# duckietown/gym-duckietown

Hardware: AMD Instinct MI355X
Metric: env-steps/sec (4096 envs, 640x480 RGB) at 1/2/4/8 MI355X; % HBM roofline (higher is better)
Workload: dtype f32 raster -> u8 frames; f64 physics

## Files before the change

gym-duckietown_amd/csrc/dtsim_dev.h:

```cpp
#pragma once
#include <hip/hip_runtime.h>
#include <stdint.h>
#include "../../include/dtsim.h"
#include "ipm_project.h"
#include "observe_plan.h"
#include "scene_tables.h"
#include "state_fields.h"

#define DT_CAMERA_FORWARD_DIST 0.066
#define DT_ROBOT_WIDTH (0.13 + 0.02)
#define DT_ROBOT_LENGTH 0.18
#define DT_CENTER_SHIFT (DT_CAMERA_FORWARD_DIST - (DT_ROBOT_LENGTH / 2))
#define DT_SAFETY_RAD_MULT 1.8
#define DT_AGENT_SAFETY_RAD ((DT_ROBOT_LENGTH / 2) * DT_SAFETY_RAD_MULT)
#define DT_REWARD_INVALID_POSE (-1000.0)

struct StepParams {
  int32_t n_steps, frame_skip, max_steps, delay_steps;
  int32_t action_mode, actions_f64, auto_reset, n_pool;
  uint32_t step_flags;
  int32_t light_capture, domain_rand;
  int32_t lanes;
  int32_t camera_rand;
  const dtsim_reset_sampler* sampler;
// ... 6 lines not shown
void dt_launch_reset(hipStream_t s, const SimArrays& A, const MapSet& M, const StepParams& P,
                     const uint8_t* mask, const dtsim_init_state* states);
void dt_launch_query(hipStream_t s, const SimArrays& A, const MapSet& M, const StepParams& P, int n,
                     const int32_t* env_idx, const double* poses, double safety_factor, dtsim_probe* out);

struct alignas(16) ScreenTri {
  float bx0, bx1, by0, by1;
  float sx[3], sy[3], iw[3];
  float inv_area;
  int32_t index;
  int32_t pad;
  float cw[3][3];
  float uw[3], vw[3];
  int32_t tex;
};
static_assert(sizeof(ScreenTri) == 128, "ScreenTri is 128 bytes");
struct ObjBox { float bx0, bx1, by0, by1; int32_t first, count, pad[2]; };

#ifndef DT_WAVE_W
#define DT_WAVE_W 128
#endif
#ifndef DT_PPT
#define DT_PPT 4
#endif
#ifndef DT_V3_WW
#define DT_V3_WW 128
#endif
#define DT_TILE_W DT_WAVE_W
#define DT_TILE_H (4 * (64 * DT_PPT / DT_WAVE_W))
#ifndef DT_ENVS_PER_BLOCK
#define DT_ENVS_PER_BLOCK 64
#endif
#ifndef DT_ITEM_B
#define DT_ITEM_B 8
#endif
#define DT_ITEMS_PER_WG (4 * (DT_PPT * DT_ENVS_PER_BLOCK) / DT_ITEM_B)
static inline size_t dt_raster_tiles(int W, int H) {
  return (size_t)((W + DT_TILE_W - 1) / DT_TILE_W) * (size_t)((H + DT_TILE_H - 1) / DT_TILE_H);
}
static inline size_t dt_raster_groups(int N, int W, int H) { return dt_raster_tiles(W, H) * (((size_t)N + DT_ENVS_PER_BLOCK - 1) / DT_ENVS_PER_BLOCK); }

struct RenderParams {
  int32_t N, W, H, distortion;
  int32_t domain_rand, n_maps, n_tile_recs;
  int32_t tex_w, tex_h;
  const TileLds* tile_recs;
  uint8_t* frames;
  const float* lut;
  const uint32_t* texels;
  const TexDev* tex;
  const RenderMapDev* maps;
  const uint32_t* tiles;
  const ObjInstDev* objs;
  const MeshDev* meshes;
  const TriDev* tris;
  void* envcam;
  int32_t max_tris, segment;
  ScreenTri* stris;
  float4* tribox;
  ObjBox* objbox;
  float* blockbox;
  unsigned long long* objmask;
  uint2* objrange;
  uint16_t* queue;
  int32_t* qcount;
  uint16_t* qend;
  int32_t* work;
  uint32_t* items;
  uint32_t* items2;
  const uint8_t* mesh_seg;
  const uint8_t* qtex;
  const uint32_t* qtiles;
  int32_t n_qtiles, qlog2;
  float q_per_m;
  int32_t qmax_tiles;
  int32_t* envpos;
  void* dump;
  void* pixtab;
  void* envv;
  void* envd;
  int32_t q3_rows;
  int32_t light;
};
#define DT_WORK_INTS 8
#define DT_WORK_ITEMS 0
#define DT_WORK_CURSOR 1
#define DT_WORK_OBJ_FRONT 2
#define DT_WORK_OBJ_CURSOR 3
#define DT_WORK_OBJ_BACK 6
#define DT_WORK_LIVE 7
struct RenderDump { uint8_t store[64 * 16]; };
enum RenderSlab { DT_SLAB_ENV, DT_SLAB_PIX, DT_SLAB_QUEUE, DT_SLAB_QCOUNT, DT_SLAB_ITEMS, DT_SLAB_QEND, DT_SLAB_STRIS, DT_SLAB_OBJBOX, DT_SLAB_OBJMASK, DT_SLABS };
void dt_render_layout(int N, int W, int H, int max_tris, size_t* bytes, void* const* base = nullptr, RenderParams* R = nullptr);
int dt_raster_pipe(RenderParams& R, int grid_rows, int grid_cols, bool raster_old);
int dt_launch_render(hipStream_t s, const SimArrays& A, const RenderParams& R, int pipe, int tables, const uint8_t* mask = nullptr);
void dt_launch_overlay_lines(hipStream_t s, const RenderParams& R, const float* d_lines, int first, int count, int env);
void dt_launch_overlay_leds(hipStream_t s, const RenderParams& R, const float* d_spheres, int first, int count, int env);
void dt_launch_depth(hipStream_t s, const RenderParams& R, void* out, int oh, int ow, bool f16, const uint8_t* mask);
void dt_launch_labels(hipStream_t s, const RenderParams& R, const uint8_t* texel_class, const uint8_t* mesh_class, int n_mesh_class, uint8_t* out,
                      uint8_t* inst, int oh, int ow, const uint8_t* mask);
void dt_launch_bev(hipStream_t s, const RenderParams& R, const SimArrays& A, const double* ocorners, const uint8_t* texel_class,
                   const uint8_t* mesh_class, int n_mesh_class, uint8_t* cls, uint8_t* inst, int oh, int ow, double cell, int rows_behind,
                   const uint8_t* mask);
struct IpmArgs {
  const uint8_t* frames;
  int N, W, H;
  uint8_t *img, *valid;
  int32_t* src;
  int oh, ow;
  double cell;
  int rows_behind;
  bool chw;
  const uint8_t* mask;
};
void dt_launch_ipm_table(hipStream_t s, int32_t* table, const IpmCal* cal, int W, int H, int oh, int ow, double cell, int rows_behind);
void dt_launch_ipm_gather(hipStream_t s, const IpmArgs& a, const int32_t* table);
void dt_launch_ipm_env(hipStream_t s, const IpmArgs& a, const SimArrays& A, bool per_env, const IpmCal* cals, int n_cal, const int32_t* env_cal);
void dt_launch_remap_cal(hipStream_t s, const uint8_t* scratch, uint8_t* frames, const int32_t* src, const int32_t* env_cal,
                         const uint8_t* mask, int N, int W, int H);
void dt_build_remap_maps(int W, int H, int n_cal, const double* K, const double* D, const double* ir, float* rx, float* ry);
void dt_fill_pack_remap(int W, int H, int n_cal, float* rx, float* ry, const int32_t* order, const int64_t* order_off, int32_t* src_index);

void dt_launch_observe(hipStream_t s, const ObservePlan& plan, const ObserveParams& P, const uint8_t* mask = nullptr);
void dt_launch_copy_rows(hipStream_t s, int N, void* dst, const void* src, size_t row_bytes, const uint8_t* mask);
void dt_launch_boxes(hipStream_t s, int N, const uint8_t* inst, int oh, int ow, int32_t* out, const uint8_t* mask);
void dt_launch_obs_push(hipStream_t s, int N, void* stack, const uint8_t* obs, int depth, int out_h, int out_w, bool f32, bool gray,
                        const uint8_t* first, const uint8_t* mask);
struct BlendArgs {
  const uint8_t* f[DTSIM_BLEND_MAX];
  uint32_t w[DTSIM_BLEND_MAX];
  int n;
};
void dt_launch_blend_frames(hipStream_t s, int N, void* out, const BlendArgs& B, size_t frame_bytes, bool f32, const uint8_t* mask);
```

gym-duckietown_amd/csrc/render.hip:

```cpp
#include "dtsim_dev.h"
#include <hip/hip_fp16.h>
#include <type_traits>
#include <algorithm>
#include <map>
#include <mutex>
#include <tuple>

typedef int v3_i32x4 __attribute__((ext_vector_type(4)));
typedef uint32_t v3_u32x3 __attribute__((ext_vector_type(3)));
__device__ void v3_buf_store_v3i32(v3_u32x3 data, v3_i32x4 rsrc, int voffset, int soffset, int aux) __asm("llvm.amdgcn.raw.buffer.store.v3i32");
typedef uint32_t v3_u32x4 __attribute__((ext_vector_type(4)));
__device__ void v3_buf_store_v4i32(v3_u32x4 data, v3_i32x4 rsrc, int voffset, int soffset, int aux) __asm("llvm.amdgcn.raw.buffer.store.v4i32");
#define V3_RSRC_W3 0x00027000
__device__ inline v3_i32x4 v3_rsrc(const void* p, uint32_t bytes) {
  v3_i32x4 r;
  r.x = (int)(uint32_t)reinterpret_cast<uintptr_t>(p); r.y = (int)((reinterpret_cast<uintptr_t>(p) >> 32) & 0xFFFFu); r.z = (int)bytes; r.w = V3_RSRC_W3;
  return r;
}


#define RB 256
#define PPT DT_PPT
#define WAVE_W DT_WAVE_W
#define SLOT_X(k, l) (((k) * 64 + (l)) % WAVE_W)
#define SLOT_Y(k, l) (((k) * 64 + (l)) / WAVE_W)
#define WAVE_PIX (64 * PPT)
#define ENVS_PER_BLOCK DT_ENVS_PER_BLOCK
#ifndef DT_TRI_CAP
#define DT_TRI_CAP 96
#endif
#ifndef DT_TRI_PAD
#define DT_TRI_PAD 0.5f
#endif
#define TRI_CAP DT_TRI_CAP

#define CLS_SKY 0
#define CLS_GROUND 1
#define CLS_TILE 2

#define NEAR_Z 0.04f
#define FAR_Z 100.0f
#define GROUND_Y (-0.008f)
#define GROUND_HALF 50.0f

struct alignas(16) EnvCam {
  float Cx, Cy, Cz;
  float sa, ca;
  float sth, cth;
  float tx, ty;
  float hor[3];
  float gnd[3];
  float base[3];
  float dif[3];
  float L[4];
  float gndl[4];
  int32_t map_id;
  float pad[2];
};
static_assert(sizeof(EnvCam) == 128, "EnvCam is 128 bytes");

struct alignas(16) EnvFast {
  float A, B, Cxi, Czi;
  float kg, Cx, Cz, its;
  float ts, gw_m, gh_m, I0;
  uint32_t hor_rgb;
  int32_t gw, gh, tile_off;
};
static_assert(sizeof(EnvFast) == 64, "EnvFast is 64 bytes");

struct alignas(16) EnvQ {
  float A, B, Cx, Cz;
  float Xhi, Zhi;
  uint32_t tab_b, pitch4;
  uint32_t hor_rgb;
  uint32_t sky[3];
  uint32_t reach;
  uint32_t env;
  uint32_t pad[2];
};
static_assert(sizeof(EnvQ) == 64, "EnvQ is 64 bytes");
struct alignas(16) EnvV {
  float A2[2], B2[2], Cx2[2], Cz2[2];
  float Xhi, Zhi;
// ... 853 lines not shown
}

__device__ inline PixInv pix_inv_dr(float nx, float ny, bool valid, const DrCam& d, const float L[4]) {
  PixInv p;
  p.flags = valid ? PF_VALID : 0u;
  p.lr = p.lf = p.ndl = p.mrg = 0.f;
  const float xe = nx * d.tx, yla = fmaf(ny, d.a1, -d.sth), fwd = fmaf(ny, d.a2, d.cth);
  if (!(yla < 0.f)) {
    p.flags |= (yla - d.dy >= 0.f) ? PF_SKY : PF_ALWAYS_EDGE;
    return p;
  }
  const float inv = frcp(-yla);
  const float t = d.Cy * inv;
  p.lr = t * xe; p.lf = t * fwd;
  if (d.directional) p.ndl = d.ndl_dir;
  else { Ray r; r.xe = xe; r.ye = ny * d.ty; r.yla = yla; r.fwd = fwd; p.ndl = plane_ndl(L, d.sth, d.cth, r, t); }
  const float rho = d.dy * inv;
  const float kappa = fmaf(rho * 1.3334f, rho, rho);
  const float sx = fmaf(fabsf(p.lr), kappa, t * d.cex), fy = fmaf(fabsf(p.lf), kappa, t * d.eys);
  p.mrg = 1.05f * fsqrt_(fmaf(sx, sx, fy * fy));
  const float tg = t * d.kgc;
  if (t >= NEAR_Z && t <= FAR_Z) p.flags |= PF_TILE_OK;
  if (tg >= NEAR_Z && tg <= FAR_Z) p.flags |= PF_GROUND_OK;
  if (rho > 0.25f || tg * (1.f + 2.f * rho) > FAR_Z * 0.98f || t * (1.f - 2.f * rho) < NEAR_Z * 1.02f)
    p.flags |= PF_ALWAYS_EDGE;
  return p;
}

#define QREGION (WAVE_PIX * ENVS_PER_BLOCK)
#define QE_PLANE_EDGE 0x8000u
__device__ inline int qe_pixel(const uint32_t ent) { return (int)(ent & 255u); }
__device__ inline int qe_envpos(const uint32_t ent) { return (int)((ent >> 8) & 63u); }
__device__ inline bool qe_plane_edge(const uint32_t ent) { return (ent & QE_PLANE_EDGE) != 0u; }
static_assert(ENVS_PER_BLOCK <= 64, "the env position of a queue entry has six bits");
#define ITEM_B DT_ITEM_B
#define ITEMS_PER_WG DT_ITEMS_PER_WG
#define GRAB_MAX 16
#ifndef DT_RES_ENVS
#define DT_RES_ENVS 1
#endif
#define RES_ENVS DT_RES_ENVS
static_assert(ENVS_PER_BLOCK % RES_ENVS == 0 && ENVS_PER_BLOCK / RES_ENVS <= ITEMS_PER_WG, "octet items");

__device__ inline int dt_sub_live(const RenderParams& R) { return __builtin_amdgcn_readfirstlane(R.work[DT_WORK_LIVE]); }
__device__ inline size_t obj_items_cap(const RenderParams& R) {
  const int n_tiles = ((R.W + DT_TILE_W - 1) / DT_TILE_W) * ((R.H + DT_TILE_H - 1) / DT_TILE_H);
  return (size_t)((R.N + ENVS_PER_BLOCK - 1) / ENVS_PER_BLOCK) * n_tiles * (ENVS_PER_BLOCK / RES_ENVS);
}
typedef unsigned long long envmask_t;
__device__ inline void push_obj_items(const RenderParams& R, uint32_t rwg, envmask_t groups = ~0ull, envmask_t heavy = 0ull) {
  const int ng = ENVS_PER_BLOCK / RES_ENVS;
  if (ng < 64) groups &= (1ull << ng) - 1ull;
  heavy &= groups;
  const envmask_t light = groups & ~heavy;
  const int nh = __popcll(heavy), nl = __popcll(light);
  if (nh) {
    int pos = atomicAdd(R.work + DT_WORK_OBJ_FRONT, nh);
    for (int i = 0; i < ng; ++i) if ((heavy >> i) & 1ull) R.items2[pos++] = rwg * ITEMS_PER_WG + (uint32_t)i;
  }
  if (nl) {
    size_t pos = obj_items_cap(R) - 1 - (size_t)atomicAdd(R.work + DT_WORK_OBJ_BACK, nl);
    for (int i = 0; i < ng; ++i) if ((light >> i) & 1ull) R.items2[pos--] = rwg * ITEMS_PER_WG + (uint32_t)i;
  }
}
#ifndef DT_RO_HEAVY
#define DT_RO_HEAVY 128
#endif
__device__ inline envmask_t obj_groups_of(int qend_v, int lane, envmask_t* heavy = nullptr) {
  static_assert(ENVS_PER_BLOCK / RES_ENVS <= 64, "one bit per env group");
  const int up = __shfl_up(qend_v, 1);
  const int cnt = lane < ENVS_PER_BLOCK ? qend_v - (lane == 0 ? 0 : up) : 0;
  const unsigned long long m = __ballot(cnt != 0), mh = __ballot(cnt >= DT_RO_HEAVY);
  envmask_t g = 0ull, gh = 0ull;
#pragma unroll
  for (int i = 0; i < ENVS_PER_BLOCK / RES_ENVS; ++i) {
    g |= ((m >> (i * RES_ENVS)) & ((1ull << RES_ENVS) - 1ull)) ? (1ull << i) : 0ull;
    gh |= ((mh >> (i * RES_ENVS)) & ((1ull << RES_ENVS) - 1ull)) ? (1ull << i) : 0ull;
  }
  if (heavy) *heavy = gh;
  return g;
}


#ifndef DT_Q_TILE_SPLIT
#define DT_Q_TILE_SPLIT 2
#endif
__host__ __device__ inline int dt_q_tile_group(int n_tiles) { return (n_tiles + DT_Q_TILE_SPLIT - 1) / DT_Q_TILE_SPLIT; }
inline size_t raster_wg_grid(size_t n_tiles, int n_chunks) {
  const int q_tg = dt_q_tile_group((int)n_tiles);
  return ((n_tiles + q_tg - 1) / q_tg) * q_tg * ((n_chunks + 7) / 8) * 8;
}
struct RasterWg {
  int NL, tile, chunk; bool live;
  __device__ int rwg(const int n_tiles) const { return chunk * n_tiles + tile; }
  __device__ int e0() const { return chunk * ENVS_PER_BLOCK; }
  __device__ int e1() const { return min(e0() + ENVS_PER_BLOCK, NL); }
};
template <bool SUB, bool SCALAR>
__device__ inline RasterWg raster_wg(const RenderParams& R, const int n_tiles, const unsigned bx) {
  RasterWg w;
  w.NL = SUB ? dt_sub_live(R) : R.N;
  const int n_chunks = (w.NL + ENVS_PER_BLOCK - 1) / ENVS_PER_BLOCK, cpx = (n_chunks + 7) / 8;
  const int xcd = bx & 7, bi = bx >> 3;
  const int q_tg = dt_q_tile_group(n_tiles);
  const int per_group = q_tg * cpx;
  const int grp = bi / per_group, gi = bi % per_group;
  const int g_tiles = min(q_tg, n_tiles - grp * q_tg);
  const int tile = SUB ? (int)bx % n_tiles : grp * q_tg + gi % g_tiles;
  w.tile = SCALAR ? __builtin_amdgcn_readfirstlane(tile) : tile;
  const int chunk = SUB ? (int)bx / n_tiles : xcd * cpx + gi / g_tiles;
  w.chunk = SCALAR ? __builtin_amdgcn_readfirstlane(chunk) : chunk;
  w.live = SUB ? w.chunk < n_chunks : (gi < g_tiles * cpx && w.chunk < n_chunks);
  return w;
}

#define V3_TAB_PITCH 256
#define V3_MAP_COLS 32
__device__ inline void v3_fill_tile_table(const RenderParams& R, const uint32_t* __restrict__ qtiles, uint32_t* s_qt, const int tid) {
  for (int i = tid; i < R.q3_rows * V3_TAB_PITCH; i += RB) s_qt[i] = 0u;
  __syncthreads();
  for (int mi = 0; mi < R.n_maps; ++mi) {
    const int pitch = R.maps[mi].qt_pitch, off = R.maps[mi].qt_off, n = pitch * (R.maps[mi].grid_h + 2 * DT_QRING);
    for (int i = tid; i < n; i += RB) {
      const int r = i / pitch, c = i - r * pitch;
      const uint2 te = reinterpret_cast<const uint2*>(qtiles)[off + i];
      s_qt[r * V3_TAB_PITCH + mi * V3_MAP_COLS + c] = te.x;
      s_qt[r * V3_TAB_PITCH + V3_TAB_PITCH / 2 + mi * V3_MAP_COLS + c] = te.y;
    }
  }
}

__device__ inline void fill_tile_recs(const RenderParams& R, uint32_t* s_mem, const int tid) {
  const uint32_t* src = reinterpret_cast<const uint32_t*>(R.tile_recs);
  for (int i = tid; i < R.n_tile_recs * (int)(sizeof(TileLds) / 4); i += RB) s_mem[i] = src[i];
}

__device__ inline float med3f(float x, float lo, float hi) { return __builtin_amdgcn_fmed3f(x, lo, hi); }
__device__ inline bool v3_sample_owner(const float Xs, const float Zs, const float lo, const float Xhi, const float Zhi, const char* qtb,
                                       const uint32_t tab, uint32_t& tb, uint32_t& sel) {
  const float Xo = Xs - 0.5f, Zo = Zs - 0.5f;
  const float Xc = med3f(Xo, lo, Xhi), Zc = med3f(Zo, lo, Zhi);
  const uint32_t ta = (__builtin_amdgcn_perm((uint32_t)flr_i32(Zc), (uint32_t)flr_i32(Xc), 0x0c0c0501u) << 2) + tab;
  const uint32_t* tp = reinterpret_cast<const uint32_t*>(qtb + ta);
  tb = tp[0]; sel = tp[V3_TAB_PITCH / 2];
  return (Xc == Xo) & (Zc == Zo);
}
__device__ inline float ground_quad_at(const float kg, const float X, const float C) { return fmaf(kg, X - C, C); }
__device__ inline bool ground_quad_in(const float G, const float goff, const float ghalf) { return fabsf(G - goff) <= ghalf; }

__device__ inline int work_n_grabs(const int n_items) {
  const int grab = max(1, min(GRAB_MAX, n_items / (int)(gridDim.x * (RB / 64) * 4)));
  return (n_items + grab - 1) / grab;
}
__device__ inline int work_next_grab(const RenderParams& R, const int cursor, int g, const int lane) {
  if (lane == 0) g = (int)gridDim.x * (RB / 64) + atomicAdd(R.work + cursor, 1);
  return __builtin_amdgcn_readfirstlane(g);
}

template <bool OBJ>
struct ChunkObjMasks {
  static_assert(ENVS_PER_BLOCK <= 64, "one lane per env of the chunk");
  uint32_t lo, hi;
  int e0;
  __device__ void load(const RenderParams& R, const int e0_, const int e1, const int n_blk, const int blk, const int lane) {
    uint32_t om_lo = 0u, om_hi = 0u;
    if (OBJ && lane < e1 - e0_) {
      const unsigned long long v = R.objmask[(size_t)(e0_ + lane) * n_blk + blk];
      om_lo = (uint32_t)v; om_hi = (uint32_t)(v >> 32);
    }
    lo = om_lo; hi = om_hi; e0 = e0_;
  }
  __device__ unsigned long long of(const int e) const {
    if (!OBJ) return 0ull;
    return ((unsigned long long)(uint32_t)__builtin_amdgcn_readlane((int)hi, e - e0) << 32) | (uint32_t)__builtin_amdgcn_readlane((int)lo, e - e0);
  }
};

__device__ inline uint32_t spxy_pack(const float4& l, const int W, const int H) {
  const float sx = (l.x + 1.f) * 0.5f * (float)W, sy = (1.f - l.y) * 0.5f * (float)H;
  return (uint32_t)__half_as_ushort(__float2half(sx)) | ((uint32_t)__half_as_ushort(__float2half(sy)) << 16);
}
__device__ inline void spxy_unpack(uint32_t t, float& sx, float& sy) {
  asm volatile("" : "+v"(t));
  sx = __half2float(__ushort_as_half((unsigned short)(t & 0xFFFFu)));
  sy = __half2float(__ushort_as_half((unsigned short)(t >> 16)));
}

struct alignas(4) U3 { uint32_t a, b, c; };

template <bool DR, bool OBJ>
__global__ __launch_bounds__(RB) void k_raster(RenderParams R, const EnvCam* __restrict__ cams,
                                               const EnvFast* __restrict__ fasts, uint8_t* __restrict__ frames, const uint32_t* __restrict__ texels,
                                               const float4* __restrict__ lut, const RenderMapDev* __restrict__ maps,
                                               const TileLds* __restrict__ tile_recs, uint16_t* __restrict__ queue,
                                               int32_t* __restrict__ qcount) {
  extern __shared__ uint32_t s_mem[];
// ... 1632 lines not shown
}

void dt_launch_ipm_env(hipStream_t s, const IpmArgs& a, const SimArrays& A, bool per_env, const IpmCal* cals, int n_cal, const int32_t* env_cal) {
  if (a.N <= 0) return;
  const bool vec = dt_ipm_vec(a);
  auto k = a.chw ? (vec ? k_ipm_env<true, true> : k_ipm_env<true, false>) : (vec ? k_ipm_env<false, true> : k_ipm_env<false, false>);
  hipLaunchKernelGGL(k, dt_ipm_grid(a), dim3(256), 0, s, a.frames, A.angle, A.cam, per_env ? 1 : 0, dt_ipm_shared_camera(a.W, a.H), cals, n_cal, env_cal,
                     a.N, a.W, a.H, a.oh, a.ow, a.cell, a.rows_behind, a.img, a.valid, a.src, a.mask);
}

void dt_launch_overlay_lines(hipStream_t s, const RenderParams& R, const float* d_lines, int first, int count, int env) {
  if (count <= 0) return;
  hipLaunchKernelGGL(k_overlay_lines, dim3((unsigned)((R.W * R.H + 255) / 256)), dim3(256), 0, s, R, reinterpret_cast<const EnvCam*>(R.envcam), d_lines, first, count, env);
}

template <class K> static size_t resident_blocks(K kernel, size_t lds) {
  static std::mutex mu;
  static std::map<std::tuple<int, size_t, const void*>, size_t> cache;
  int dev = 0;
  (void)hipGetDevice(&dev);
  std::lock_guard<std::mutex> lk(mu);
  const auto key = std::make_tuple(dev, lds, reinterpret_cast<const void*>(kernel));
  auto it = cache.find(key);
  if (it != cache.end()) return it->second;
  int per_cu = 0, n_cu = 0;
  if (hipOccupancyMaxActiveBlocksPerMultiprocessor(&per_cu, kernel, RB, lds) != hipSuccess || per_cu < 1) per_cu = 3;
  if (hipDeviceGetAttribute(&n_cu, hipDeviceAttributeMultiprocessorCount, dev) != hipSuccess || n_cu < 1) n_cu = 256;
  return cache[key] = (size_t)per_cu * (size_t)n_cu;
}

#define DT_SCRATCH_ALIGN 64
static_assert(DT_SCRATCH_ALIGN % 64 == 0 && DT_SCRATCH_ALIGN % alignof(EnvD) == 0 && DT_SCRATCH_ALIGN % alignof(float4) == 0,
              "EnvQ, EnvV and EnvD records are 64-byte aligned (one scalar load each), tribox 16-byte aligned (float4)");
struct Slab {
  char* base; size_t bytes = 0;
  template <class T> T* take(size_t n) {
    const size_t off = (bytes + DT_SCRATCH_ALIGN - 1) / DT_SCRATCH_ALIGN * DT_SCRATCH_ALIGN;
    bytes = off + n * sizeof(T); return base ? reinterpret_cast<T*>(base + off) : nullptr;
  }
};
struct EnvRecs { EnvCam* cams; EnvFast* fasts; EnvQ* envq; EnvV* envv; EnvD* envd; EnvL* envl; PixTab* pixtab; SampTab* samptab; };
static EnvRecs render_layout(int N, int W, int H, int max_tris, size_t* bytes, void* const* base, RenderParams& R) {
  const size_t n = (size_t)N, n_pix = (size_t)W * H, n_tiles = dt_raster_tiles(W, H), n_wg = dt_raster_groups(N, W, H);
  Slab sl[DT_SLABS];
  for (int i = 0; i < DT_SLABS; ++i) sl[i].base = base ? static_cast<char*>(base[i]) : nullptr;
  Slab &env = sl[DT_SLAB_ENV], &pix = sl[DT_SLAB_PIX], &qc = sl[DT_SLAB_QCOUNT], &it = sl[DT_SLAB_ITEMS], &ob = sl[DT_SLAB_OBJMASK];
  EnvRecs x;
  R.envcam = x.cams = env.take<EnvCam>(n); x.fasts = env.take<EnvFast>(n); x.envq = env.take<EnvQ>(n); R.envpos = env.take<int32_t>(n);
  R.envv = x.envv = env.take<EnvV>(n + 1); R.envd = x.envd = env.take<EnvD>(n); x.envl = env.take<EnvL>(n + 1);
  R.pixtab = x.pixtab = pix.take<PixTab>(n_pix); x.samptab = pix.take<SampTab>(n_pix); R.dump = pix.take<RenderDump>(1);
  R.queue = sl[DT_SLAB_QUEUE].take<uint16_t>(n_wg * (RB / 64) * QREGION);
  R.qcount = qc.take<int32_t>(n_wg * (RB / 64)); R.work = qc.take<int32_t>(DT_WORK_INTS);
  R.items = it.take<uint32_t>(n_wg * ITEMS_PER_WG); R.items2 = it.take<uint32_t>(n_wg * ENVS_PER_BLOCK);
  R.qend = sl[DT_SLAB_QEND].take<uint16_t>(n_wg * (RB / 64) * ENVS_PER_BLOCK);
  if (max_tris > 0) {
    R.stris = sl[DT_SLAB_STRIS].take<ScreenTri>(n * max_tris); R.tribox = sl[DT_SLAB_STRIS].take<float4>(n * max_tris);
    R.objbox = sl[DT_SLAB_OBJBOX].take<ObjBox>(n * DTSIM_MAX_OBJECTS);
    R.blockbox = reinterpret_cast<float*>(ob.take<float4>(n_tiles * 4)); R.objrange = ob.take<uint2>((size_t)DTSIM_MAX_MAPS * DTSIM_MAX_OBJECTS);
    R.objmask = ob.take<unsigned long long>(n * n_tiles * 4);
  }
  if (bytes) for (int i = 0; i < DT_SLABS; ++i) bytes[i] = sl[i].bytes;
  return x;
}
void dt_render_layout(int N, int W, int H, int max_tris, size_t* bytes, void* const* base, RenderParams* R) { RenderParams tmp{}; render_layout(N, W, H, max_tris, bytes, base, R ? *R : tmp); }

int dt_raster_pipe(RenderParams& R, int grid_rows, int grid_cols, bool raster_old) {
  const bool v3 = R.qlog2 == 8 && grid_rows <= V3_MAX_ROWS && grid_cols <= V3_MAP_COLS && R.n_maps * V3_MAP_COLS <= V3_TAB_PITCH / 2 && !raster_old;
  R.q3_rows = v3 ? grid_rows : 0;
  const bool records = R.qtex && !R.segment && (R.W & 3) == 0;
  if (records && !R.domain_rand && (size_t)R.n_qtiles * 8 <= 32768 && !(R.qlog2 == 8 && R.qmax_tiles >= 256)) return v3 ? DTSIM_PIPE_V3 : DTSIM_PIPE_Q;
  if (records && R.domain_rand && v3) return DTSIM_PIPE_V3DR;
  return (R.domain_rand || R.segment || R.light) ? DTSIM_PIPE_GENERIC_ENV : DTSIM_PIPE_GENERIC;
}

template <bool SUB>
static void launch_raster_resolve(hipStream_t s, const RenderParams& R, const EnvRecs& x, int pipe, bool has_pos) {
  const bool obj = R.max_tris > 0, quad = pipe == DTSIM_PIPE_V3 || pipe == DTSIM_PIPE_Q;
  const int n_chunks = (R.N + ENVS_PER_BLOCK - 1) / ENVS_PER_BLOCK;
  const size_t lds = (size_t)R.n_tile_recs * sizeof(TileLds);
  const size_t lds1 = lds + (size_t)RB * PPT * sizeof(uint32_t);
  const size_t lds2 = lds + (size_t)(RB / 64) * ENVS_PER_BLOCK * sizeof(EnvCam);
  const dim3 grid((unsigned)(dt_raster_tiles(R.W, R.H) * n_chunks));
  const dim3 gridq((unsigned)raster_wg_grid(dt_raster_tiles(R.W, R.H), n_chunks));
  const size_t ldsq = (size_t)R.n_qtiles * 8 + (size_t)RB * PPT * sizeof(uint32_t);
  const size_t lds_tab = (size_t)R.q3_rows * V3_TAB_PITCH * 4;
  const size_t lds3 = lds_tab + (size_t)(RB / 64) * V3_WAVE_LDS * 4 + (size_t)ENVS_PER_BLOCK * sizeof(EnvQ);
  const size_t ldsd = lds_tab + (size_t)(RB / 64) * RQ_LIST * 4;
  const bool s256 = R.qlog2 == 8 && R.qmax_tiles < 256;
#define LAUNCH_RASTER(DR_, OBJ_)                                                                              \
  hipLaunchKernelGGL((k_raster<DR_, OBJ_>), grid, dim3(RB), lds1, s, R, x.cams, x.fasts, R.frames, R.texels,                  \
                     reinterpret_cast<const float4*>(R.lut), R.maps, R.tile_recs, R.queue, R.qcount)
#define LAUNCH_Q(OBJ_, S256_) do { if (R.light) hipLaunchKernelGGL((k_raster_q<OBJ_, S256_, true, SUB>), gridq, dim3(RB), ldsq, s, R, x.cams, x.fasts, x.envq, R.frames, \
                                           R.qtex, reinterpret_cast<const float4*>(R.lut), x.pixtab, x.samptab, R.qtiles, R.queue, R.qcount, x.envl); \
                                else hipLaunchKernelGGL((k_raster_q<OBJ_, S256_, false, SUB>), gridq, dim3(RB), ldsq, s, R, x.cams, x.fasts, x.envq, R.frames, R.qtex, \
                                           reinterpret_cast<const float4*>(R.lut), x.pixtab, x.samptab, R.qtiles, R.queue, R.qcount, nullptr); } while (0)
#define LAUNCH_V3(OBJ_) do { if (R.light) hipLaunchKernelGGL((k_raster_v3<OBJ_, true, SUB>), gridq, dim3(RB), lds3, s, R, x.cams, x.fasts, x.envq, x.envv, R.frames, \
                                           R.qtex, reinterpret_cast<const float4*>(R.lut), x.pixtab, x.samptab, R.qtiles, R.queue, R.qcount, x.envl); \
                                else hipLaunchKernelGGL((k_raster_v3<OBJ_, false, SUB>), gridq, dim3(RB), lds3, s, R, x.cams, x.fasts, x.envq, x.envv, R.frames, R.qtex, \
                                           reinterpret_cast<const float4*>(R.lut), x.pixtab, x.samptab, R.qtiles, R.queue, R.qcount, nullptr); } while (0)
  switch (pipe) {
    case DTSIM_PIPE_V3: if (obj) LAUNCH_V3(true); else LAUNCH_V3(false); break;
    case DTSIM_PIPE_Q: if (obj) { if (s256) LAUNCH_Q(true, true); else LAUNCH_Q(true, false); } else if (s256) LAUNCH_Q(false, true); else LAUNCH_Q(false, false); break;
    case DTSIM_PIPE_V3DR:
      if (obj) hipLaunchKernelGGL((k_raster_v3dr<true, SUB>), gridq, dim3(RB), ldsd, s, R, x.cams, x.envd, R.frames, R.qtex, reinterpret_cast<const float4*>(R.lut), R.qtiles, R.queue, R.qcount);
      else hipLaunchKernelGGL((k_raster_v3dr<false, SUB>), gridq, dim3(RB), ldsd, s, R, x.cams, x.envd, R.frames, R.qtex, reinterpret_cast<const float4*>(R.lut), R.qtiles, R.queue, R.qcount);
      break;
    case DTSIM_PIPE_GENERIC_ENV: if (obj) LAUNCH_RASTER(true, true); else LAUNCH_RASTER(true, false); break;
    default: if (obj) LAUNCH_RASTER(false, true); else LAUNCH_RASTER(false, false);
  }
#undef LAUNCH_V3
#undef LAUNCH_Q
#undef LAUNCH_RASTER
  if (pipe == DTSIM_PIPE_V3DR) {
    const dim3 rgrid((unsigned)std::min<size_t>(grid.x, resident_blocks(k_resolve_dr, lds_tab)));
    hipLaunchKernelGGL(k_resolve_dr, rgrid, dim3(RB), lds_tab, s, R, x.cams, x.envd, R.qtex, reinterpret_cast<const float4*>(R.lut), R.qtiles, R.queue, R.qcount);
  } else if (!quad) {
    const dim3 rgrid((unsigned)std::min<size_t>(grid.x, resident_blocks(k_resolve, lds2)));
    hipLaunchKernelGGL(k_resolve, rgrid, dim3(RB), lds2, s, R, x.cams, R.queue, R.qcount);
  }
  if (obj) {
    const size_t lds4 = lds + (size_t)(RB / 64) * TRI_CAP * sizeof(TriCov) + (size_t)(RB / 64) * RO_SCR_BYTES;
    const dim3 rgrid((unsigned)std::min<size_t>(grid.x, resident_blocks(k_resolve_obj<DT_RES_NB>, lds4)));
    hipLaunchKernelGGL(k_resolve_obj<DT_RES_NB>, rgrid, dim3(RB), lds4, s, R, x.cams, R.queue, has_pos ? x.envq : (const EnvQ*)nullptr);
  }
}

int dt_launch_render(hipStream_t s, const SimArrays& A, const RenderParams& R_in, int pipe, int tables, const uint8_t* mask) {
  RenderParams R = R_in;
  tables &= 3;
  void* base[DT_SLABS] = {R.envcam, R.pixtab}; RenderParams carved{};
  const EnvRecs x = render_layout(A.N, R.W, R.H, 0, nullptr, base, carved);
  const bool quad = pipe == DTSIM_PIPE_V3 || pipe == DTSIM_PIPE_Q, v3dr = pipe == DTSIM_PIPE_V3DR;
  int32_t* pos = ((quad || v3dr) && R.envpos && A.N > ENVS_PER_BLOCK) ? R.envpos : nullptr;
  const bool sub = mask && (quad || v3dr) && R.envpos;
  if (sub) {
    pos = R.envpos;
    (void)hipMemsetAsync(R.work, 0, DT_WORK_INTS * sizeof(int32_t), s);
    hipLaunchKernelGGL(k_env_sort<true>, dim3(1), dim3(1024), 0, s, A, R.maps, pos, mask, R.work + DT_WORK_LIVE);
    tables |= 4;
  } else if (pos) { hipLaunchKernelGGL(k_env_sort<false>, dim3(1), dim3(1024), 0, s, A, R.maps, pos, nullptr, nullptr); tables |= 4; }
#define LAUNCH_CAM(M_) hipLaunchKernelGGL(k_cam_setup<M_>, dim3((A.N + 63) / 64), dim3(64), 0, s, A, R.domain_rand, R.segment,                  \
                     (float)R.W / (float)R.H, x.cams, x.fasts, R.maps, (quad || v3dr) ? x.envq : nullptr, R.qlog2, pos, quad ? x.envv : nullptr,  \
                     v3dr ? x.envd : nullptr, R.W, R.H, R.light, (quad && R.light) ? x.envl : nullptr)
  if (sub) LAUNCH_CAM(true); else LAUNCH_CAM(false);
#undef LAUNCH_CAM
  if (!sub) (void)hipMemsetAsync(R.work, 0, DT_WORK_INTS * sizeof(int32_t), s);
  if (R.max_tris > 0) {
    if (!(tables & 2)) hipLaunchKernelGGL(k_blk_setup, dim3((unsigned)dt_raster_tiles(R.W, R.H)), dim3(RB), 0, s, R, reinterpret_cast<const float4*>(R.lut), reinterpret_cast<float4*>(R.blockbox));
    tables |= 2;
    if (sub) hipLaunchKernelGGL(k_obj_setup<true>, dim3(A.N), dim3(DT_OBJSETUP_T), 0, s, A, R, x.cams, pos);
    else hipLaunchKernelGGL(k_obj_setup<false>, dim3(A.N), dim3(DT_OBJSETUP_T), 0, s, A, R, x.cams, pos);
  }

  if (quad && !(tables & 1)) {
    hipLaunchKernelGGL(k_pix_setup, dim3((R.W * R.H + 255) / 256), dim3(256), 0, s, R, reinterpret_cast<const float4*>(R.lut), x.pixtab, x.samptab);
    tables |= 1;
  }
  if (sub) launch_raster_resolve<true>(s, R, x, pipe, true);
  else launch_raster_resolve<false>(s, R, x, pipe, pos != nullptr);
  return tables;
}
```

gym-duckietown_amd/csrc/render_v3.inc:

```

#ifndef DT_V3_WAVES
#define DT_V3_WAVES 6
#endif
#ifndef DT_V3_WAVES_OBJ
#define DT_V3_WAVES_OBJ (DT_V3_WAVES - 1)
#endif
#define DT_V3_SW (DT_V3_WW / 4)
#define V3_ROWS (WAVE_PIX / DT_V3_WW)
#define V3_WX (DT_TILE_W / DT_V3_WW)
static_assert(PPT == 4 && DT_V3_WW == 128 && DT_V3_WW == WAVE_W && DT_TILE_W % DT_V3_WW == 0 && (RB / 64) % V3_WX == 0 &&
              V3_ROWS * ((RB / 64) / V3_WX) == DT_TILE_H, "k_raster_v3 / k_raster_v3dr: 128 x 2 wavefront blocks tiling the 128 x 8 workgroup tile "
              "(the generic k_resolve / k_resolve_obj decode the queue entries as row-major pixel numbers of such a block)");
#define V3_MAX_ROWS 24
#define V3_SEL_TILE 0x0c0c0602u
#define V3_WAVE_LDS RQ_LIST
static_assert(DT_V3_WW == 4 * DT_V3_SW && 64 % DT_V3_SW == 0, "four slots side by side");
#define V3_PIX(k, l) (((l) / DT_V3_SW) * DT_V3_WW + (k) * DT_V3_SW + ((l) % DT_V3_SW))
#define V3_XP_LANE(l) (((l) / DT_V3_SW) * DT_V3_WW + ((l) % DT_V3_SW))
#define V3_XO1 "96"
#define V3_XO1G "97"
#define V3_XO1B "98"
#define V3_XO2 "192"
#define V3_XO2G "193"
#define V3_XO2B "194"
// ... 26 lines not shown
      const int lp = qe_pixel(ent), el = qe_envpos(ent);
      const int pix = have ? (by0 + lp / DT_V3_WW) * R.W + bx0 + lp % DT_V3_WW : 0;
      const SampTab sp = samptab[pix];
      PixTab pt;
      pt.lr = __uint_as_float(sp.pad[0]); pt.lf = __uint_as_float(sp.pad[1]); pt.lit = __uint_as_float(sp.pad[2]); pt.mi = 0u;
      const uint4* fl = s_envq + el * 4;
      const uint4 a4 = fl[0];
      const float4 qa = make_float4(__uint_as_float(a4.x), __uint_as_float(a4.y), __uint_as_float(a4.z), __uint_as_float(a4.w));
      const uint4 qb = fl[1], qd = fl[3];
      const float A = qa.x, B = qa.y, Cx = qa.z, Cz = qa.w, Xhi = __uint_as_float(qb.x), Zhi = __uint_as_float(qb.y);
      const uint32_t tab = qd.z;
      const int e = (int)qd.y;
      const float4* c4 = reinterpret_cast<const float4*>(cams + e);
      const float wCy = default_cam((float)R.W / (float)R.H).Cy;
      const float kg = (wCy - GROUND_Y) / wCy;
      const float qpm = __uint_as_float(qd.w);
      const float goff = (float)DT_QRING * Sf + 0.5f, ghalf = GROUND_HALF * qpm;
      const float Xu = fmaf(pt.lf, B, fmaf(pt.lr, A, Cx)), Zu = fmaf(pt.lf, -A, fmaf(pt.lr, B, Cz));
      const uint32_t xic = q8_bits(Xu), zic = q8_bits(Zu);
      float lit8 = (pt.lit > 0.f ? pt.lit : 0.55f) * Q8_LIT;
      if constexpr (LIGHT) { if (pt.lit > 0.f) lit8 = env_lit8(envl[min(e0 + el, R.N - 1)], pt.lr, pt.lf, env_base8()); }
      const uint32_t W8 = quad_weights8(q8_frac(xic), q8_frac(zic), lit8);
      uint32_t aS[3] = {0u, 0u, 0u};
      int n_sky = 0, n_gnd = 0;
      float gX = 0.f, gZ = 0.f;
      uint4 rec = make_uint4(0u, 0u, 0u, 0u);
      uint32_t raddr_prev = 0u;
#pragma unroll
      for (int s = 3; s >= 0; --s) {
        const uint32_t hr = sp.dlr[s >> 1], hf = sp.dlf[s >> 1];
        const float slr = pt.lr + __half2float(__ushort_as_half((unsigned short)((s & 1) ? hr >> 16 : hr)));
        const float slf = pt.lf + __half2float(__ushort_as_half((unsigned short)((s & 1) ? hf >> 16 : hf)));
        const float Xs = fmaf(slf, B, fmaf(slr, A, Cx)), Zs = fmaf(slf, -A, fmaf(slr, B, Cz));
        uint32_t tb, sel;
        const bool s_in = v3_sample_owner(Xs, Zs, lo, Xhi, Zhi, qtb, tab, tb, sel);
        const bool is_tile = have & (((sp.flags >> s) & 1u) != 0u) & s_in & (tb != 0u);
        const float Xg = ground_quad_at(kg, Xs, Cx), Zg = ground_quad_at(kg, Zs, Cz);
        const bool is_gnd = have & !is_tile & (((sp.flags >> (4 + s)) & 1u) != 0u) & ground_quad_in(Xg, goff, ghalf) & ground_quad_in(Zg, goff, ghalf);
        n_gnd += is_gnd; n_sky += !(is_tile | is_gnd);
        if (is_gnd) { gX = Xg; gZ = Zg; }
        const uint32_t raddr = is_tile ? (tb | q8_rec256(xic, zic, sel)) : 0u;
        if (s == 3 || raddr != raddr_prev) rec = *reinterpret_cast<const uint4*>(qtex + raddr);
        raddr_prev = raddr;
        aS[0] = __builtin_amdgcn_udot4(rec.x, W8, aS[0], false);
        aS[1] = __builtin_amdgcn_udot4(rec.y, W8, aS[1], false);
        aS[2] = __builtin_amdgcn_udot4(rec.z, W8, aS[2], false);
      }
      float acc[3];
      float4 hc = make_float4(0.f, 0.f, 0.f, 0.f);
      if (__ballot(n_sky > 0)) hc = c4[2];
      acc[0] = fmaf((float)n_sky, hc.y, (float)aS[0] * (1.f / 256.f));
      acc[1] = fmaf((float)n_sky, hc.z, (float)aS[1] * (1.f / 256.f));
      acc[2] = fmaf((float)n_sky, hc.w, (float)aS[2] * (1.f / 256.f));
      if (__ballot(n_gnd > 0)) {
        if (pt.lit > 0.f && (pt.lr != 0.f || pt.lf != 0.f)) { gX = fmaf(kg, Xu - Cx, Cx); gZ = fmaf(kg, Zu - Cz, Cz); }
        const float hs = 0.5f / ghalf;
        const float a_ = fminf(fmaxf(fmaf(gX - goff, hs, 0.5f), 0.f), 1.f), b_ = fminf(fmaxf(fmaf(gZ - goff, hs, 0.5f), 0.f), 1.f);
        const float4 q3 = c4[3], q4 = c4[4], q5 = c4[5], q6 = c4[6], q7 = c4[7];
        const float ndl = ground_corner_ndl(a_, b_, q6.y, q6.z, q6.w, q7.x);
        const float ng = (float)n_gnd;
        acc[0] += ng * ground_lit(q3.x, q3.w, q4.z, ndl);
        acc[1] += ng * ground_lit(q3.y, q4.x, q4.w, ndl);
        acc[2] += ng * ground_lit(q3.z, q4.y, q5.x, ndl);
      }
      const float o[3] = {0.25f * acc[0], 0.25f * acc[1], 0.25f * acc[2]};
      if (have) store_rgb(R.frames, npix, e, pix, pack_rgb(o));
    }
    __builtin_amdgcn_fence(__ATOMIC_RELEASE, "wavefront");
    __builtin_amdgcn_wave_barrier();
  }
}

template <bool OBJ, bool LIGHT = false, bool SUB = false>
__global__ __launch_bounds__(RB) __attribute__((amdgpu_waves_per_eu(OBJ ? DT_V3_WAVES_OBJ : DT_V3_WAVES, OBJ ? DT_V3_WAVES_OBJ : DT_V3_WAVES)))
void k_raster_v3(RenderParams R, const EnvCam* __restrict__ cams, const EnvFast* __restrict__ fasts, const EnvQ* __restrict__ envq,
                 const EnvV* __restrict__ envv, uint8_t* __restrict__ frames, const uint8_t* __restrict__ qtex, const float4* __restrict__ lut,
                 const PixTab* __restrict__ pixtab, const SampTab* __restrict__ samptab, const uint32_t* __restrict__ qtiles,
                 uint16_t* __restrict__ queue, int32_t* __restrict__ qcount, const EnvL* __restrict__ envl) {
  extern __shared__ uint32_t s_mem[];
  uint32_t* s_qt = s_mem;
  const int tid = threadIdx.x;
  const int npix = R.W * R.H;
  const int tiles_x = (R.W + DT_TILE_W - 1) / DT_TILE_W, n_tiles = tiles_x * ((R.H + DT_TILE_H - 1) / DT_TILE_H);
  const RasterWg wg = raster_wg<SUB, true>(R, n_tiles, blockIdx.x);
  if (!wg.live) return;
  const int NL = wg.NL, tile = wg.tile, rwg = wg.rwg(n_tiles), e0 = wg.e0(), e1 = wg.e1();
  v3_fill_tile_table(R, qtiles, s_qt, tid);
  uint4* s_envq = reinterpret_cast<uint4*>(s_mem + R.q3_rows * V3_TAB_PITCH + (RB / 64) * V3_WAVE_LDS);
  static_assert(ENVS_PER_BLOCK * 4 <= RB, "one 16-byte piece per thread");
  if (tid < ENVS_PER_BLOCK * 4) s_envq[tid] = reinterpret_cast<const uint4*>(envq + min(e0 + tid / 4, NL - 1))[tid & 3];
  __syncthreads();

  const int wave = __builtin_amdgcn_readfirstlane(tid >> 6), lane = tid & 63;
  const int bx0 = (tile % tiles_x) * DT_TILE_W + (wave % V3_WX) * DT_V3_WW;
  const int by0 = (tile / tiles_x) * DT_TILE_H + (wave / V3_WX) * V3_ROWS;
  const float lo = 0.5f * 256.f;

  float lr[PPT], lf[PPT], lit[PPT];
  uint32_t Mi[PPT];
  bool cand[PPT], gok[PPT], valid[PPT];
  uint32_t spxy[PPT];
#pragma unroll
  for (int k = 0; k < PPT; ++k) {
    PixTab t{0.f, 0.f, -1.f, 0xFFFFu};
    const int x = bx0 + V3_PIX(k, lane) % DT_V3_WW, y = by0 + V3_PIX(k, lane) / DT_V3_WW;
    const bool inimg = x < R.W && y < R.H;
    if (inimg) t = pixtab[y * R.W + x];
    lr[k] = t.lr; lf[k] = t.lf; lit[k] = fmaxf(t.lit, 0.f) * Q8_LIT; Mi[k] = t.mi;
    valid[k] = t.lit >= 0.f; cand[k] = t.lit > 0.f; gok[k] = (t.mi & 0xFFFFu) != 0xFFFFu;
    spxy[k] = 0u;
    if (OBJ && inimg) spxy[k] = spxy_pack(lut[y * R.W + x], R.W, R.H);
  }
  bool any_cand = false;
#pragma unroll
  for (int k = 0; k < PPT; ++k) any_cand |= cand[k];

  uint16_t* w_queue = queue + ((size_t)rwg * (RB / 64) + wave) * QREGION;
  int qn = 0, qo = 0;
  int qend_v = 0;
  uint32_t* w_lds = s_mem + R.q3_rows * V3_TAB_PITCH + wave * V3_WAVE_LDS;
  const int st_x = bx0 + (lane * 4) % DT_V3_WW, st_y = by0 + (lane * 4) / DT_V3_WW;
  const bool st_ok = st_x < R.W && st_y < R.H;
  const size_t st_off = ((size_t)st_y * R.W + st_x) * 3;

  ChunkObjMasks<OBJ> objmasks;
  objmasks.load(R, e0, e1, n_tiles * 4, tile * 4 + wave, lane);
  auto push_obj = [&](const int e, const uint32_t env, unsigned long long om, unsigned long long oem[PPT], const unsigned long long em[PPT]) __attribute__((always_inline)) {
    const ObjBox* boxes = R.objbox + (size_t)env * DTSIM_MAX_OBJECTS;
    bool oedge[PPT];
#pragma unroll
    for (int k = 0; k < PPT; ++k) oedge[k] = false;
    const float obj_mrg = (R.W > 2048 || R.H > 2048) ? 0.95f : (R.W > 1024 || R.H > 1024) ? 0.45f : 0.3f;
    float sx[PPT], sy[PPT];
#pragma unroll
    for (int k = 0; k < PPT; ++k) spxy_unpack(spxy[k], sx[k], sy[k]);
    while (om) {
      const int o = __builtin_ctzll(om);
      const ObjBox ob = boxes[o];
      om &= om - 1ull;
#pragma unroll
      for (int k = 0; k < PPT; ++k)
        if (valid[k] && sx[k] >= ob.bx0 - obj_mrg && sx[k] <= ob.bx1 + obj_mrg && sy[k] >= ob.by0 - obj_mrg && sy[k] <= ob.by1 + obj_mrg) oedge[k] = true;
    }
    bool any_oedge = false;
#pragma unroll
    for (int k = 0; k < PPT; ++k) any_oedge |= oedge[k];
    if (__ballot(any_oedge)) {
      const uint32_t etag = (uint32_t)(e - e0) << 8;
#pragma unroll
      for (int k = 0; k < PPT; ++k) {
        const bool ek = oedge[k];
        const unsigned long long mk = __ballot(ek);
        oem[k] = mk;
        if (ek) {
          const int rank = __builtin_amdgcn_mbcnt_hi((uint32_t)(mk >> 32), __builtin_amdgcn_mbcnt_lo((uint32_t)mk, 0u));
          w_queue[QREGION - 1 - (qo + rank)] = (uint16_t)(etag | (__builtin_amdgcn_inverse_ballot_w64(em[k]) ? QE_PLANE_EDGE : 0u) | (uint32_t)V3_PIX(k, lane));
        }
        qo += __popcll(mk);
      }
    }
  };
  const uint32_t st_voff = st_ok ? (uint32_t)st_off : 0x80000000u;
  const uint32_t frame_bytes = (uint32_t)npix * 3u;
  const bool wide = __builtin_amdgcn_readfirstlane((int)(R.W % DT_V3_WW == 0 && R.H % V3_ROWS == 0)) != 0;
  const uint32_t st_voff16 = lane < 48 ? (uint32_t)(((size_t)(by0 + lane / V3_ROW16) * R.W + bx0) * 3u) + (uint32_t)(lane % V3_ROW16) * 16u : 0x80000000u;
  auto store = [&](const uint32_t env, const U4& o) __attribute__((always_inline)) {
    const v3_i32x4 fr = v3_rsrc(frames + (size_t)env * frame_bytes, frame_bytes);
    if (wide) v3_buf_store_v4i32(v3_u32x4{o.a, o.b, o.c, o.d}, fr, (int)st_voff16, 0, 2);
    else v3_buf_store_v3i32(v3_u32x3{o.a, o.b, o.c}, fr, (int)st_voff, 0, 2);
  };
// ... 262 lines not shown
```

Measured before the change: 2.797 million.

## Add per-XCD ticket work stealing for the tail of the v3 raster grid

Moves the tile/chunk mapping of the raster grid into a shared header. It then makes the last items of each XCD's list claimable through per-XCD atomic ticket counters held in the work buffer. Extra 'thief' workgroups are launched so that idle workgroups can take leftover items from other XCDs, aiming to even out tail imbalance. The cost is atomics, an extra barrier and a larger grid, and work may now run on an XCD away from its L2-local data.

```diff
diff --git a/gym-duckietown_amd/csrc/dtsim_dev.h b/gym-duckietown_amd/csrc/dtsim_dev.h
--- a/gym-duckietown_amd/csrc/dtsim_dev.h
+++ b/gym-duckietown_amd/csrc/dtsim_dev.h
@@ -112,13 +112,14 @@
   int32_t q3_rows;
   int32_t light;
 };
-#define DT_WORK_INTS 8
+#define DT_WORK_INTS (32 + 8 * 32)
 #define DT_WORK_ITEMS 0
 #define DT_WORK_CURSOR 1
 #define DT_WORK_OBJ_FRONT 2
 #define DT_WORK_OBJ_CURSOR 3
 #define DT_WORK_OBJ_BACK 6
 #define DT_WORK_LIVE 7
+#define DT_WORK_TICKETS 32
 struct RenderDump { uint8_t store[64 * 16]; };
 enum RenderSlab { DT_SLAB_ENV, DT_SLAB_PIX, DT_SLAB_QUEUE, DT_SLAB_QCOUNT, DT_SLAB_ITEMS, DT_SLAB_QEND, DT_SLAB_STRIS, DT_SLAB_OBJBOX, DT_SLAB_OBJMASK, DT_SLABS };
 void dt_render_layout(int N, int W, int H, int max_tris, size_t* bytes, void* const* base = nullptr, RenderParams* R = nullptr);
diff --git a/gym-duckietown_amd/csrc/raster_map.h b/gym-duckietown_amd/csrc/raster_map.h
--- /dev/null
+++ b/gym-duckietown_amd/csrc/raster_map.h
@@ -0,0 +1,88 @@
+#pragma once
+#include <stddef.h>
+
+#if defined(__HIPCC__)
+#define DT_MAP_FN __host__ __device__ inline
+#else
+#define DT_MAP_FN inline
+#endif
+
+#ifndef DT_Q_TILE_SPLIT
+#define DT_Q_TILE_SPLIT 2
+#endif
+#define DT_RASTER_XCDS 8
+DT_MAP_FN int dt_q_tile_group(int n_tiles) { return (n_tiles + DT_Q_TILE_SPLIT - 1) / DT_Q_TILE_SPLIT; }
+DT_MAP_FN int raster_cpx(int n_chunks) { return (n_chunks + DT_RASTER_XCDS - 1) / DT_RASTER_XCDS; }
+inline size_t raster_wg_grid(size_t n_tiles, int n_chunks) {
+  const int q_tg = dt_q_tile_group((int)n_tiles);
+  return ((n_tiles + q_tg - 1) / q_tg) * q_tg * ((n_chunks + 7) / 8) * 8;
+}
+
+struct RasterItem { int tile, chunk; bool live; };
+DT_MAP_FN int raster_list_slots(int n_tiles, int n_chunks) {
+  const int q_tg = dt_q_tile_group(n_tiles);
+  return (n_tiles + q_tg - 1) / q_tg * q_tg * raster_cpx(n_chunks);
+}
+DT_MAP_FN RasterItem raster_item(int n_tiles, int n_chunks, int xcd, int k) {
+  const int cpx = raster_cpx(n_chunks);
+  const int q_tg = dt_q_tile_group(n_tiles);
+  const int per_group = q_tg * cpx;
+  const int grp = k / per_group, gi = k % per_group;
+  const int g_tiles = q_tg < n_tiles - grp * q_tg ? q_tg : n_tiles - grp * q_tg;
+  RasterItem it;
+  it.tile = grp * q_tg + gi % g_tiles;
+  it.chunk = xcd * cpx + gi / g_tiles;
+  it.live = gi < g_tiles * cpx && it.chunk < n_chunks;
+  return it;
+}
+
+DT_MAP_FN int raster_list_chunks(int n_chunks, int xcd) {
+  const int cpx = raster_cpx(n_chunks), left = n_chunks - xcd * cpx;
+  return left < 0 ? 0 : left < cpx ? left : cpx;
+}
+DT_MAP_FN int raster_list_len(int n_tiles, int n_chunks, int xcd) { return n_tiles * raster_list_chunks(n_chunks, xcd); }
+DT_MAP_FN int raster_live_index(int n_tiles, int n_chunks, int xcd, int k) {
+  const int q_tg = dt_q_tile_group(n_tiles), per_group = q_tg * raster_cpx(n_chunks);
+  return k / per_group * q_tg * raster_list_chunks(n_chunks, xcd) + k % per_group;
+}
+DT_MAP_FN RasterItem raster_live_item(int n_tiles, int n_chunks, int xcd, int j) {
+  const int q_tg = dt_q_tile_group(n_tiles), per_group = q_tg * raster_list_chunks(n_chunks, xcd);
+  const int grp = j / per_group, gi = j % per_group;
+  const int g_tiles = q_tg < n_tiles - grp * q_tg ? q_tg : n_tiles - grp * q_tg;
+  RasterItem it;
+  it.tile = grp * q_tg + gi % g_tiles;
+  it.chunk = xcd * raster_cpx(n_chunks) + gi / g_tiles;
+  it.live = true;
+  return it;
+}
+
+#define DT_TICKET_LAST_GROUP (-1)
+#define DT_TICKET_ALL (-2)
+#ifndef DT_RASTER_TICKET_UNITS
+#define DT_RASTER_TICKET_UNITS 1
+#endif
+#define DT_TICKET_STRIDE 32
+DT_MAP_FN int raster_ticket_len(int n_tiles, int n_chunks, int xcd, int units) {
+  const int len = raster_list_len(n_tiles, n_chunks, xcd);
+  const int q_tg = dt_q_tile_group(n_tiles), g_last = n_tiles - (n_tiles - 1) / q_tg * q_tg;
+  if (units == DT_TICKET_ALL) return len;
+  if (units == DT_TICKET_LAST_GROUP) return g_last * raster_list_chunks(n_chunks, xcd);
+  return units * g_last < len ? units * g_last : len;
+}
+DT_MAP_FN bool raster_slot_static(int n_tiles, int n_chunks, int xcd, int k, int units) {
+  if (k >= raster_list_slots(n_tiles, n_chunks)) return false;
+  if (!raster_item(n_tiles, n_chunks, xcd, k).live) return false;
+  return raster_live_index(n_tiles, n_chunks, xcd, k) < raster_list_len(n_tiles, n_chunks, xcd) - raster_ticket_len(n_tiles, n_chunks, xcd, units);
+}
+DT_MAP_FN int raster_thieves(int n_tiles, int n_chunks, int units) {
+  int most = 0;
+  for (int x = 0; x < DT_RASTER_XCDS; ++x) { const int s = raster_ticket_len(n_tiles, n_chunks, x, units); most = s > most ? s : most; }
+  return units == DT_TICKET_ALL ? 0 : most;
+}
+inline size_t raster_ticket_grid(size_t n_tiles, int n_chunks, int units) { return raster_wg_grid(n_tiles, n_chunks) + (size_t)DT_RASTER_XCDS * raster_thieves((int)n_tiles, n_chunks, units); }
+DT_MAP_FN int raster_claim_xcd(int xcd, int attempt) { return (xcd + attempt) & (DT_RASTER_XCDS - 1); }
+DT_MAP_FN RasterItem raster_ticket_item(int n_tiles, int n_chunks, int x, int t, int units) {
+  const int s = raster_ticket_len(n_tiles, n_chunks, x, units);
+  if (t >= s) return RasterItem{0, 0, false};
+  return raster_live_item(n_tiles, n_chunks, x, raster_list_len(n_tiles, n_chunks, x) - s + t);
+}
diff --git a/gym-duckietown_amd/csrc/render.hip b/gym-duckietown_amd/csrc/render.hip
--- a/gym-duckietown_amd/csrc/render.hip
+++ b/gym-duckietown_amd/csrc/render.hip
@@ -1,4 +1,5 @@
 #include "dtsim_dev.h"
+#include "raster_map.h"
 #include <hip/hip_fp16.h>
 #include <type_traits>
 #include <algorithm>
@@ -1018,36 +1019,56 @@
 }
 
 
-#ifndef DT_Q_TILE_SPLIT
-#define DT_Q_TILE_SPLIT 2
-#endif
-__host__ __device__ inline int dt_q_tile_group(int n_tiles) { return (n_tiles + DT_Q_TILE_SPLIT - 1) / DT_Q_TILE_SPLIT; }
-inline size_t raster_wg_grid(size_t n_tiles, int n_chunks) {
-  const int q_tg = dt_q_tile_group((int)n_tiles);
-  return ((n_tiles + q_tg - 1) / q_tg) * q_tg * ((n_chunks + 7) / 8) * 8;
-}
 struct RasterWg {
-  int NL, tile, chunk; bool live;
+  int NL, tile, chunk; bool live, claims, thief;
   __device__ int rwg(const int n_tiles) const { return chunk * n_tiles + tile; }
   __device__ int e0() const { return chunk * ENVS_PER_BLOCK; }
   __device__ int e1() const { return min(e0() + ENVS_PER_BLOCK, NL); }
 };
-template <bool SUB, bool SCALAR>
+template <bool SUB, bool SCALAR, bool TICKET = false>
 __device__ inline RasterWg raster_wg(const RenderParams& R, const int n_tiles, const unsigned bx) {
+  static_assert(!(SUB && TICKET), "the masked pass keeps its linear map");
   RasterWg w;
   w.NL = SUB ? dt_sub_live(R) : R.N;
-  const int n_chunks = (w.NL + ENVS_PER_BLOCK - 1) / ENVS_PER_BLOCK, cpx = (n_chunks + 7) / 8;
+  const int n_chunks = (w.NL + ENVS_PER_BLOCK - 1) / ENVS_PER_BLOCK;
   const int xcd = bx & 7, bi = bx >> 3;
-  const int q_tg = dt_q_tile_group(n_tiles);
-  const int per_group = q_tg * cpx;
-  const int grp = bi / per_group, gi = bi % per_group;
-  const int g_tiles = min(q_tg, n_tiles - grp * q_tg);
-  const int tile = SUB ? (int)bx % n_tiles : grp * q_tg + gi % g_tiles;
+  const bool thief = TICKET && bi >= raster_list_slots(n_tiles, n_chunks);
+  const RasterItem it = raster_item(n_tiles, n_chunks, xcd, thief ? 0 : bi);
+  const int tile = SUB ? (int)bx % n_tiles : it.tile;
   w.tile = SCALAR ? __builtin_amdgcn_readfirstlane(tile) : tile;
-  const int chunk = SUB ? (int)bx / n_tiles : xcd * cpx + gi / g_tiles;
+  const int chunk = SUB ? (int)bx / n_tiles : it.chunk;
   w.chunk = SCALAR ? __builtin_amdgcn_readfirstlane(chunk) : chunk;
-  w.live = SUB ? w.chunk < n_chunks : (gi < g_tiles * cpx && w.chunk < n_chunks);
+  w.live = SUB ? w.chunk < n_chunks : (it.live && !thief);
+  w.claims = TICKET && __builtin_amdgcn_readfirstlane((int)(thief || !raster_slot_static(n_tiles, n_chunks, xcd, thief ? 0 : bi, DT_RASTER_TICKET_UNITS))) != 0;
+  w.thief = thief;
   return w;
+}
+static_assert(DT_WORK_TICKETS >= DT_TICKET_STRIDE && DT_WORK_TICKETS + DT_RASTER_XCDS * DT_TICKET_STRIDE <= DT_WORK_INTS, "the ticket counters lie inside R.work (zeroed before every pass)");
+__device__ inline int raster_claim_issue(const RenderParams& R, const unsigned bx, const int tid, const RasterWg& w) {
+  if (w.thief) return 0x7fffffff;
+  return tid == 0 ? atomicAdd(R.work + DT_WORK_TICKETS + (int)(bx & 7) * DT_TICKET_STRIDE, 1) : 0;
+}
+__device__ inline void raster_claim_finish(const RenderParams& R, const int n_tiles, const unsigned bx, const int first, int* s_claim, const int tid, RasterWg& w) {
+  const int n_chunks = (w.NL + ENVS_PER_BLOCK - 1) / ENVS_PER_BLOCK;
+  if (tid == 0) {
+    RasterItem it = raster_ticket_item(n_tiles, n_chunks, (int)(bx & 7), first, DT_RASTER_TICKET_UNITS);
+    if (!it.live) {
+      int seen[DT_RASTER_XCDS];
+#pragma unroll
+      for (int a = 1; a < DT_RASTER_XCDS; ++a)
+        seen[a] = __hip_atomic_load(R.work + DT_WORK_TICKETS + raster_claim_xcd((int)(bx & 7), a) * DT_TICKET_STRIDE, __ATOMIC_RELAXED, __HIP_MEMORY_SCOPE_AGENT);
+#pragma unroll
+      for (int a = 1; a < DT_RASTER_XCDS; ++a) {
+        const int x = raster_claim_xcd((int)(bx & 7), a);
+        if (it.live || seen[a] >= raster_ticket_len(n_tiles, n_chunks, x, DT_RASTER_TICKET_UNITS)) continue;
+        it = raster_ticket_item(n_tiles, n_chunks, x, atomicAdd(R.work + DT_WORK_TICKETS + x * DT_TICKET_STRIDE, 1), DT_RASTER_TICKET_UNITS);
+      }
+    }
+    s_claim[0] = it.live ? it.tile : -1; s_claim[1] = it.chunk;
+  }
+  __syncthreads();
+  w.tile = __builtin_amdgcn_readfirstlane(s_claim[0]); w.chunk = __builtin_amdgcn_readfirstlane(s_claim[1]);
+  w.live = w.tile >= 0;
 }
 
 #define V3_TAB_PITCH 256
@@ -2846,6 +2867,7 @@
   const size_t lds2 = lds + (size_t)(RB / 64) * ENVS_PER_BLOCK * sizeof(EnvCam);
   const dim3 grid((unsigned)(dt_raster_tiles(R.W, R.H) * n_chunks));
   const dim3 gridq((unsigned)raster_wg_grid(dt_raster_tiles(R.W, R.H), n_chunks));
+  const dim3 gridv3(SUB ? gridq.x : (unsigned)raster_ticket_grid(dt_raster_tiles(R.W, R.H), n_chunks, DT_RASTER_TICKET_UNITS));
   const size_t ldsq = (size_t)R.n_qtiles * 8 + (size_t)RB * PPT * sizeof(uint32_t);
   const size_t lds_tab = (size_t)R.q3_rows * V3_TAB_PITCH * 4;
   const size_t lds3 = lds_tab + (size_t)(RB / 64) * V3_WAVE_LDS * 4 + (size_t)ENVS_PER_BLOCK * sizeof(EnvQ);
@@ -2858,9 +2880,9 @@
                                            R.qtex, reinterpret_cast<const float4*>(R.lut), x.pixtab, x.samptab, R.qtiles, R.queue, R.qcount, x.envl); \
                                 else hipLaunchKernelGGL((k_raster_q<OBJ_, S256_, false, SUB>), gridq, dim3(RB), ldsq, s, R, x.cams, x.fasts, x.envq, R.frames, R.qtex, \
                                            reinterpret_cast<const float4*>(R.lut), x.pixtab, x.samptab, R.qtiles, R.queue, R.qcount, nullptr); } while (0)
-#define LAUNCH_V3(OBJ_) do { if (R.light) hipLaunchKernelGGL((k_raster_v3<OBJ_, true, SUB>), gridq, dim3(RB), lds3, s, R, x.cams, x.fasts, x.envq, x.envv, R.frames, \
+#define LAUNCH_V3(OBJ_) do { if (R.light) hipLaunchKernelGGL((k_raster_v3<OBJ_, true, SUB>), gridv3, dim3(RB), lds3, s, R, x.cams, x.fasts, x.envq, x.envv, R.frames, \
                                            R.qtex, reinterpret_cast<const float4*>(R.lut), x.pixtab, x.samptab, R.qtiles, R.queue, R.qcount, x.envl); \
-                                else hipLaunchKernelGGL((k_raster_v3<OBJ_, false, SUB>), gridq, dim3(RB), lds3, s, R, x.cams, x.fasts, x.envq, x.envv, R.frames, R.qtex, \
+                                else hipLaunchKernelGGL((k_raster_v3<OBJ_, false, SUB>), gridv3, dim3(RB), lds3, s, R, x.cams, x.fasts, x.envq, x.envv, R.frames, R.qtex, \
                                            reinterpret_cast<const float4*>(R.lut), x.pixtab, x.samptab, R.qtiles, R.queue, R.qcount, nullptr); } while (0)
   switch (pipe) {
     case DTSIM_PIPE_V3: if (obj) LAUNCH_V3(true); else LAUNCH_V3(false); break;
diff --git a/gym-duckietown_amd/csrc/render_v3.inc b/gym-duckietown_amd/csrc/render_v3.inc
--- a/gym-duckietown_amd/csrc/render_v3.inc
+++ b/gym-duckietown_amd/csrc/render_v3.inc
@@ -132,10 +132,16 @@
   const int tid = threadIdx.x;
   const int npix = R.W * R.H;
   const int tiles_x = (R.W + DT_TILE_W - 1) / DT_TILE_W, n_tiles = tiles_x * ((R.H + DT_TILE_H - 1) / DT_TILE_H);
-  const RasterWg wg = raster_wg<SUB, true>(R, n_tiles, blockIdx.x);
-  if (!wg.live) return;
+  RasterWg wg = raster_wg<SUB, true, !SUB>(R, n_tiles, blockIdx.x);
+  if (!wg.live && !wg.claims) return;
+  int* s_claim = reinterpret_cast<int*>(s_mem + R.q3_rows * V3_TAB_PITCH);
+  const int ticket = wg.claims ? raster_claim_issue(R, blockIdx.x, tid, wg) : 0;
+  v3_fill_tile_table(R, qtiles, s_qt, tid);
+  if (wg.claims) {
+    raster_claim_finish(R, n_tiles, blockIdx.x, ticket, s_claim, tid, wg);
+    if (!wg.live) return;
+  }
   const int NL = wg.NL, tile = wg.tile, rwg = wg.rwg(n_tiles), e0 = wg.e0(), e1 = wg.e1();
-  v3_fill_tile_table(R, qtiles, s_qt, tid);
   uint4* s_envq = reinterpret_cast<uint4*>(s_mem + R.q3_rows * V3_TAB_PITCH + (RB / 64) * V3_WAVE_LDS);
   static_assert(ENVS_PER_BLOCK * 4 <= RB, "one 16-byte piece per thread");
   if (tid < ENVS_PER_BLOCK * 4) s_envq[tid] = reinterpret_cast<const uint4*>(envq + min(e0 + tid / 4, NL - 1))[tid & 3];
```

Result: no change. 2.855 million (median of 6 runs) (+2.0%).
